# fishaudio/Bert-VITS2

Hardware: AMD Instinct MI355X
Metric: audio-seconds/sec (44.1 kHz), SynthesizerTrn.infer(), 128-phoneme utterance (higher is better)
Workload: dtype f32; 1 GPU; BASELINE config 2: B=1 x T=128 symbols per GPU, fp32 Generator (split-bf16 MFMA), fp32 flow, fp32 text encoder / durations / spline; utterances_per_gpu=1, symbols=128, frames=384, parallelism=utterance-sharded x1, hipgraph=False, hip_force_dev_kernarg=1

## Files before the change

### bert-vits2_amd/csrc/bv2_kernels.h

```cpp
#pragma once
#include <hip/hip_runtime_api.h>
#include <stdint.h>
#include <map>
#include <mutex>
#include <utility>

namespace bv2 {

#if defined(__HIPCC__)
__device__ __forceinline__ bool xcd_decode(unsigned id, int per, int B, int& b, int& r) {
  const unsigned slot = id >> 3;
  b = (int)(slot / (unsigned)per) * 8 + (int)(id & 7u);
  r = (int)(slot % (unsigned)per);
  return b < B;
}
#endif
inline int xcd_grid(int B, int per) { return 8 * ((B + 7) / 8) * per; }

struct Prefetch { const void* ptr; unsigned bytes; };
constexpr int PF_BLOCKS = 128;
#if defined(__HIPCC__)
__device__ __forceinline__ void prefetch_tail(const Prefetch pf, unsigned l, unsigned j, unsigned tid, unsigned nthreads) {
  const unsigned lines = (pf.bytes + 127u) >> 7;
  const unsigned lx = (lines + 7u) >> 3;
// ... 53 lines not shown
  int act;
  int mask_pre;
  int res_mode;
  int mask_post;
  const uint16_t* w3;
  const float* w3inv;
  const unsigned* xmax;
  unsigned* omax;
};

#define BV2_MAX_PROBS 8
#define BV2_MAX_KSPLIT 8
struct ConvLaunch {
  ConvProb p[BV2_MAX_PROBS];
  int nprob;
  int B;
  int L;
  const int64_t* lens = nullptr; int len_mul = 1;
  int ksplit;
  int64_t slab_stride;
  unsigned long long* dbg = nullptr;
  Prefetch pf = {nullptr, 0};
  int no_head = 0;
};

struct ConvLaunch1 {
  ConvProb p;
  int L; int64_t slab_stride; unsigned long long* dbg;
};
struct SkHead {
  const float* x; const float* w; const float* in_mask;
  int x_rstride, Lin, ntiles, per_xcd, total;
  unsigned pk0, pk1;
};
struct SkSmall { int k, dil, pad_left, ksplit, cin, cin_pad; };
#if defined(__HIPCC__)
#define BV2_HD __host__ __device__
#else
#define BV2_HD
#endif
BV2_HD inline SkSmall sk_head_unpack(unsigned pk0, unsigned pk1) {
  return SkSmall{(int)(pk0 & 255u), (int)((pk0 >> 8) & 255u), (int)((pk0 >> 16) & 255u), (int)(pk0 >> 24), (int)(pk1 & 65535u), (int)(pk1 >> 16)};
}
inline bool sk_head_pack(const ConvLaunch& L, int ntiles, int per_xcd, int total, SkHead* h) {
  const ConvProb& p = L.p[0];
  if (L.no_head || L.nprob != 1 || L.B != 1 || L.lens || p.nsrc != 1 || (L.pf.ptr && L.pf.bytes)) return false;
  if (p.k < 1 || p.k > 255 || p.dil < 1 || p.dil > 255 || p.pad_left < 0 || p.pad_left > 255 || L.ksplit < 1 || L.ksplit > 255) return false;
  if (p.cin < 1 || p.cin > 65535 || p.cin_pad < 1 || p.cin_pad > 65535) return false;
  h->x = p.x[0]; h->w = p.w; h->in_mask = p.in_mask;
  h->x_rstride = p.x_rstride; h->Lin = p.Lin; h->ntiles = ntiles; h->per_xcd = per_xcd; h->total = total;
  h->pk0 = (unsigned)p.k | (unsigned)p.dil << 8 | (unsigned)p.pad_left << 16 | (unsigned)L.ksplit << 24;
  h->pk1 = (unsigned)p.cin | (unsigned)p.cin_pad << 16;
  return true;
}
void conv_set_timeline(unsigned long long* dev_buf, long long capacity_u64);
int conv_timeline_report(long long* meta, int max_launches);
unsigned long long* timeline_slice(unsigned gx, unsigned gy, unsigned gz, int tile, int ks, int cin, int L);

enum { TILE_AUTO = 0, TILE_128x128 = 1, TILE_64x128 = 2, TILE_64x64 = 3, TILE_32x128 = 4, TILE_32x256 = 5, TILE_SPLITK = 6, TILE_128x64 = 7,
       TILE_X6 = 8,
       TILE_X6_128x64 = 9, TILE_X6_128x64_LD = 10, TILE_X6_64x128 = 11, TILE_X6_32x256 = 12,
       TILE_X3 = 14 };
int launch_conv1d(hipStream_t stream, const ConvLaunch& L, int tile, const char** variant_name);
enum { PLACE_PLAIN = 0, PLACE_PER_XCD = 1, PLACE_SNAKE = 2 };
void conv_note_placement(int place);
int conv_last_placement();
inline int64_t x6_w_index(int j, int ci, int co, int cin, int k, int plane) {
  const int64_t U = (int64_t)(cin / 16) * k, u = (int64_t)(ci / 16) * k + j;
  const int lane = (co & 31) + 32 * ((ci % 16) / 8);
  return ((((int64_t)(co >> 5) * U + u) * 3 + plane) * 64 + lane) * 8 + (ci % 8);
}
inline int64_t x6_w_elems(int cin, int cout_pad, int k) { return (int64_t)(cout_pad / 32) * (cin / 16) * k * 3 * 512; }
inline uint16_t f2bf(float f) {
  uint32_t u;
  __builtin_memcpy(&u, &f, 4);
  if ((u & 0x7fffffffu) > 0x7f800000u) return (uint16_t)((u >> 16) | 0x40u);
  u += 0x7fffu + ((u >> 16) & 1u);
  return (uint16_t)(u >> 16);
}
inline uint16_t f2h(float f) {
  const _Float16 h = (_Float16)f;
  uint16_t u;
  __builtin_memcpy(&u, &h, 2);
  return u;
}
inline float h2f(uint16_t u) {
  _Float16 h;
  __builtin_memcpy(&h, &u, 2);
  return (float)h;
}
inline void x6_split(float v, uint16_t h[3]) {
  for (int p = 0; p < 3; ++p) {
    uint32_t u;
    __builtin_memcpy(&u, &v, 4);
    uint16_t b;
    if ((u & 0x7fffffffu) > 0x7f800000u) b = (uint16_t)((u >> 16) | 0x40u);
    else if (p == 0 && (u & 0x7fffffffu) > 0x7f7f0000u) b = (uint16_t)((u >> 16) & 0x8000u) | 0x7f7fu;
    else { u += 0x7fffu + ((u >> 16) & 1u); b = (uint16_t)(u >> 16); }
    h[p] = b;
// ... 512 lines not shown
```

### bert-vits2_amd/csrc/bv2_testing.cpp

```cpp
#include <cmath>
#include <cstddef>
#include <cstring>
#include <vector>

#include "bv2_internal.h"
#include "bv2_pack.h"
#include "../../include/bv2_testing.h"
#include "kernels/rng.h"

using namespace bv2;

static auto t_dense(const float* w, int cin, int k) {
  return [=](int co, int ci, int j) { return w[((size_t)co * cin + ci) * k + j]; };
}
static auto t_bias(const float* b) { return [=](int co) { return b ? b[co] : 0.f; }; }

extern "C" {

int64_t bv2_test_conv_pack_floats(int cin, int cout, int k) {
  const ConvW c = conv_desc(cin, cout, k);
  const int64_t base = conv_w_floats(c) + c.cout_pad + 2048;
  return base + (cin % 32 == 0 ? x6_w_floats(c) + 64 + 2 * X3_SLOT_WORDS + x3_region_floats(c) + 64 : 0);
}
void bv2_test_x6_split(float v, uint16_t* h3) { x6_split(v, h3); }
// ... 507 lines not shown
                          float* out, int B, int H, int D, int T, int P, int span) {
  DebertaAttnArgs a;
  a.qkv = qkv; a.ld = ld; a.mask = mask; a.pk = pk; a.pq = pq; a.tab = tab; a.out = out;
  a.B = B; a.H = H; a.D = D; a.T = T; a.P = P; a.span = span;
  return launch_deberta_attn(static_cast<hipStream_t>(stream), a);
}

int bv2_test_bert_ln(void* stream, const float* a, int nslab, int64_t slab_stride, const float* gamma, const float* beta, float eps,
                     const float* mask, float* out, int B, int C, int T, const void* pf_ptr, unsigned pf_bytes) {
  BertLnArgs l;
  l.a = a; l.nslab = nslab; l.slab_stride = slab_stride; l.gamma = gamma; l.beta = beta; l.eps = eps; l.mask = mask; l.out = out;
  l.B = B; l.C = C; l.T = T;
  l.pf = Prefetch{pf_ptr, pf_bytes};
  return launch_bert_ln(static_cast<hipStream_t>(stream), l);
}

int bv2_test_bert_embed_ln(void* stream, const int64_t* input_ids, const int64_t* token_type_ids, const float* word, const float* pos,
                           const float* type, const int64_t* lengths, const float* gamma, const float* beta, float eps, float* out,
                           int B, int S, int C, int vocab, int max_pos, int type_vocab, const void* pf_ptr, unsigned pf_bytes) {
  BertEmbedArgs e;
  e.input_ids = input_ids; e.token_type_ids = token_type_ids; e.word = word; e.pos = pos; e.type = type; e.lengths = lengths;
  e.gamma = gamma; e.beta = beta; e.eps = eps; e.out = out;
  e.B = B; e.S = S; e.C = C; e.vocab = vocab; e.max_pos = max_pos; e.type_vocab = type_vocab;
  e.pf = Prefetch{pf_ptr, pf_bytes};
  return launch_bert_embed_ln(static_cast<hipStream_t>(stream), e);
}

void bv2_test_conv_timeline(void* dev_buf, long long capacity_u64) {
  conv_set_timeline(static_cast<unsigned long long*>(dev_buf), capacity_u64);
}
int bv2_test_conv_timeline_report(long long* meta, int max_launches) { return conv_timeline_report(meta, max_launches); }

void bv2_test_set_tuning(int splitk_waves, int force_ck, long tile_target) { conv_set_tuning(splitk_waves, force_ck, tile_target); }
void bv2_test_set_x6_tuning(int t256, int t128, int t64, int ck) { conv_x6_set_tuning(t256, t128, t64, ck); }
void bv2_test_x6_occupancy(int* out4) { conv_x6_occupancy(out4); }
void bv2_test_set_variants(const char* cl_spec, int cl_generic, int hc_generic) {
  conv_cl_set_tuning(cl_spec, cl_generic);
  conv_f16_set_tuning(hc_generic);
}

int64_t bv2_test_dds_pack_floats(int C) {
  return 10 * (int64_t)C + 2 * bv2_test_conv_pack_floats(C, C, 1);
}

int bv2_test_dds_layer(void* stream, const float* x, const float* pre_w_host, const float* pre_b_host, const float* z, int z_src,
                       const float* g, const float* mask, const float* dww_host, const float* dwb_host, const float* g1_host,
                       const float* b1_host, const float* g2_host, const float* b2_host, const float* w_host,
                       const float* bias_host, float* out, int dil, int last_mask, const float* post_w_host,
                       const float* post_b_host, int post_cout, float* post_out, float* zio, int z_dst, float* wpack_dev,
                       int B, int C, int T) {
  try {
    const int64_t one = bv2_test_conv_pack_floats(C, C, 1);
    std::vector<float> pk((size_t)bv2_test_dds_pack_floats(C), 0.f);
    size_t o = 0;
    auto put = [&](const float* src, size_t n) { size_t at = o; if (src) std::memcpy(&pk[o], src, n * sizeof(float)); o += n; return at; };
    const size_t o_dww = put(dww_host, 3 * (size_t)C), o_dwb = put(dwb_host, C), o_g1 = put(g1_host, C), o_b1 = put(b1_host, C),
                 o_g2 = put(g2_host, C), o_b2 = put(b2_host, C), o_pw = put(pre_w_host, C), o_pb = put(pre_b_host, C);
    const size_t o_w = o, boff = (size_t)conv_w_floats(conv_desc(C, C, 1));
    t_pack_conv(&pk[o_w], w_host, bias_host, C, C, 1, false);
    const size_t o_p = o_w + (size_t)one;
    if (post_w_host) {
      pack_f32(&pk[o_p], C, post_cout, 1, t_dense(post_w_host, C, 1));
      if (post_b_host) pack_bias(&pk[o_p + boff], post_cout, t_bias(post_b_host));
    }
    if (hipMemcpy(wpack_dev, pk.data(), sizeof(float) * pk.size(), hipMemcpyHostToDevice) != hipSuccess) return -6;
    DdsArgs a;
// ... 193 lines not shown
```

### bert-vits2_amd/csrc/kernels/attention.hip

```cpp
#include <hip/hip_runtime.h>
#include <type_traits>
#include <math.h>
#include "device_helpers.h"

namespace bv2 {

constexpr int AQ_WIDE = 32;
constexpr int AQ_NARROW = 16;
constexpr int AK = 32;
constexpr int ATTN_CUS = 256;
constexpr int AMAXW = 8;
constexpr int ANS = 4;


struct AttnHead { const float* qkv; const float* mask; const float* erv; int ld, T, H, W, ksplit; };

template <int DT, int NW, bool F16, bool ONE, bool KV16, int QT>
__device__ __forceinline__ void attention_tile(const AttnHead Hd, const AttnArgs& A, const int b, const int h, const int bx,
                                               const unsigned long long ts0) {
  static_assert(!KV16 || F16, "fp16 K / V only feed the fp16 matrix products");
  static_assert(QT == AQ_WIDE || (QT == AQ_NARROW && !F16), "the fp16 forms stay on 32 queries");
  constexpr int D = 32 * DT;
  constexpr int NT = 64 * NW;
  constexpr int AQ = QT, QSH = QT == 32 ? 5 : 4;
// ... 602 lines not shown
  if (ntiles <= 8 && !(DT == 4 && qt == AQ_NARROW)) return launch_attn_variant<DT, 8, true>(stream, a, grid, qt);
  if constexpr (DT == 4) return launch_attn_variant<DT, 4, false>(stream, a, grid, qt);
  else return launch_attn_variant<DT, 8, false>(stream, a, grid, qt);
}

int attention_pick_qtile(int B, int H, int T, int D, int ksplit, bool f16) {
  if (f16 || D < 32 || D > 128 || D % 32) return AQ_WIDE;
  const int ks = ksplit > 1 ? ksplit : 1, qtiles = (T + AQ_WIDE - 1) / AQ_WIDE;
  return (long)B * H * qtiles * ks * 2 <= ATTN_CUS ? AQ_NARROW : AQ_WIDE;
}

int launch_attention(hipStream_t stream, const AttnArgs& a) {
  if (a.W > AMAXW || a.W < 0 || a.T < 1 || a.B < 1 || a.H < 1 || a.ld % 32 || a.ld < a.T) return -1;
  if ((a.kh != nullptr) != (a.vh != nullptr) || (a.kh && !a.f16)) return -1;
  if (a.wo && (a.f16 || !a.o_out || a.Co < 1 || a.wo_groups * 8 < a.H * a.D)) return -1;
  if ((a.qtile != 0 && a.qtile != AQ_NARROW && a.qtile != AQ_WIDE) || (a.qtile == AQ_NARROW && a.f16)) return -1;
  const int ks = a.ksplit > 1 ? a.ksplit : 1;
  const int ntiles_all = (a.T + AK - 1) / AK;
  if (ks > 1 && (!a.wo || !a.ml_out || a.bo || a.res || ks > ntiles_all)) return -1;
  const int qt = a.qtile ? a.qtile : attention_pick_qtile(a.B, a.H, a.T, a.D, ks, a.f16 != 0);
  dim3 grid(((a.T + qt - 1) / qt) * ks, a.H, a.B);
  const int ntiles = (ntiles_all + ks - 1) / ks;
  switch (a.D) {
    case 32: return launch_attn_d<1>(stream, a, grid, ntiles, qt);
    case 64: return launch_attn_d<2>(stream, a, grid, ntiles, qt);
    case 96: return launch_attn_d<3>(stream, a, grid, ntiles, qt);
    case 128: return launch_attn_d<4>(stream, a, grid, ntiles, qt);
    default: return -2;
  }
}

int attention_pick_ksplit(int B, int H, int T, int max_slabs) {
  const int ntiles = (T + AK - 1) / AK;
  if (ntiles <= 8 || H < 1 || (H & (H - 1))) return 1;
  int ks = 1;
  auto wgs = [&](int k) {
    const int qt = attention_pick_qtile(B, H, T, 32, k, false);
    return (long)B * H * ((T + qt - 1) / qt) * k;
  };
  while (ks * 4 < ntiles && H * ks * 2 <= max_slabs && H * ks * 2 <= 8 && wgs(ks * 2) <= 512) ks *= 2;
  return ks;
}

double attention_flops(const AttnArgs& a) {
  return (double)a.B * a.H * (4.0 * a.T * (double)a.T * a.D);
}

}
```

### bert-vits2_amd/csrc/kernels/conv_mfma.hip

```cpp
#include <hip/hip_runtime.h>
#include "device_helpers.h"

namespace bv2 {

template <int WM, int WN, int MI, int NI, int CK, int XS>
__global__ void __launch_bounds__(256) conv1d_mfma_kernel(const ConvLaunch L, const int mtiles, const int per_xcd, const int snake_n) {
  constexpr int BM = WM * MI * 32;
  constexpr int BN = WN * NI * 32;
  constexpr int XP = XS * 64;
  constexpr int RPW = CK / 4;
  constexpr int GR = CK / 8;
  static_assert(WM * WN == 4, "4 waves per workgroup");
  extern __shared__ __attribute__((aligned(16))) float smem[];

  int pz = blockIdx.z, by = blockIdx.y, bx = blockIdx.x;
  if (snake_n > 0) {
    const int xcd = blockIdx.x & 7, pp = blockIdx.x >> 3;
    if (pp >= snake_n) return;
    const int r = pp >> 5, cc = pp & 31;
    const int rem = snake_n - (r << 5) < 32 ? snake_n - (r << 5) : 32;
    const int sidx = (r << 5) + ((r & 1) ? rem - 1 - cc : cc);
    const int per_prob = per_xcd * mtiles * L.B;
    pz = sidx / per_prob;
    const int rest = sidx - pz * per_prob;
// ... 245 lines not shown
        }
#pragma unroll
        for (int r = 0; r < 16; ++r) {
          const int dr = (r & 3) + 8 * (r >> 2);
          float v = acc[mi][ni][r] + bsum(r);
          if (act == ACT_RELU) v = v < 0.f ? 0.f : v;
          else if (act == ACT_GELU) v = 0.5f * v * (1.0f + erff(v * 0.70710678118654752440f));
          if (mask_pre) v *= om;
          if (res_mode == RES_ADD) v += rv[r];
          else if (res_mode == RES_RSUB) v = rv[r] - v;
          if (mask_post) v *= om;
          if (colok && row0 + dr < cout) {
            outb[off0 + (unsigned)dr * o_rs] = v;
            vmx = fmaxf(vmx, fabsf(v));
          }
        }
      }
    }
    if (omax_w) x3_publish(omax_w, omax_seen, vmx, lane);
  }
  if (L.dbg && tid == 0) {
    __builtin_amdgcn_s_waitcnt(0);
    unsigned long long* d = L.dbg + 8ull * (snake_n > 0 ? (unsigned long long)blockIdx.x
                                                        : ((unsigned long long)blockIdx.z * gridDim.y + blockIdx.y) * gridDim.x + blockIdx.x);
    timeline_record(d, ts0, ts1, ts2, k);
  }
}

constexpr int SK_PD = 8;


constexpr int SK_XP = 64;
constexpr int SK_RPW = 32;
struct SkTile {
  int nt, z, mt, b, ksplit;
  const float* xp; const float* mp; const float* wp;
  int x_rstride, Lin, k, dil, pad_left, cin, cin_pad;
};

template <bool MASK, int NWV, bool LDSX>
__device__ __forceinline__ void splitk_tile(float* const red_raw, const SkTile S, const ConvProb& P, const int L_L, const int64_t slab_stride,
                                            unsigned long long* const dbg, const unsigned long long ts0) {
  float (*red)[32][33] = reinterpret_cast<float (*)[32][33]>(red_raw);
  unsigned long long ts1 = 0, ts2 = 0;
  const int nt = S.nt, z = S.z, mt = S.mt, b = S.b;
  const int m0 = mt * 32, t0 = nt * 32;

  const int tid = threadIdx.x;
  const int lane = tid & 63;
  const int wid = __builtin_amdgcn_readfirstlane(tid >> 6);
  const int l31 = lane & 31, lh = lane >> 5;
  const int k = S.k, dil = S.dil, cin = S.cin, Lin = S.Lin;
  const int groups = S.cin_pad / 8;
  const float* const xp = S.xp;
  const float* const mp = MASK ? S.mp : nullptr;
  const float* const wp = S.wp;
  const unsigned x_rs4 = 4u * (unsigned)S.x_rstride;
  const unsigned w_tap = 1024u;
  const unsigned w_unit = w_tap * (unsigned)k;
  const unsigned w_lane = 16u * (unsigned)(lh * 32 + l31) + (unsigned)mt * (unsigned)groups * w_unit;
  const unsigned nsl = (unsigned)(S.ksplit * NWV), sl = (unsigned)(z * NWV + wid);
  const int g0 = (int)(((unsigned)groups * sl) / nsl), g1 = (int)(((unsigned)groups * (sl + 1u)) / nsl);
  const int U = (g1 - g0) * k;

  f32x16 acc, acc2;
#pragma unroll
  for (int r = 0; r < 16; ++r) { acc[r] = 0.f; acc2[r] = 0.f; }

  const int tcol = t0 + l31 - S.pad_left;
  f32x4 ar[SK_PD];
  float br[SK_PD][4];
  float mr[SK_PD];
  bool vmr[SK_PD];
// ... 5 lines not shown
    const int gc = g < groups ? g : groups - 1;
    return (unsigned)(8 * gc + lh) * x_rs4;
  };
  auto weight_off = [&](int g) __attribute__((always_inline)) {
    const int gc = g < groups ? g : groups - 1;
    return w_lane + (unsigned)gc * w_unit;
  };
  unsigned goff = group_off(lg), woff = weight_off(lg), joff = 0;
  auto load_unit = [&](int slot) __attribute__((always_inline)) {
    ar[slot] = ld_off4(wp, woff + joff);
    if (LDSX) {
      joff += w_tap;
      if (++lj == k) { lj = 0; joff = 0; ++lg; woff = weight_off(lg); }
      return;
    }
    const int t = tcol + lj * dil;
    const bool tok = t >= 0 && t < Lin;
    const unsigned tcl = 4u * (unsigned)(t < 0 ? 0 : (t >= Lin ? Lin - 1 : t));
    vmr[slot] = tok;
    mr[slot] = MASK ? ld_off(mp, tcl) : 1.f;
    unsigned ro = goff;
#pragma unroll
    for (int q = 0; q < 4; ++q) {
      const unsigned rc = ro < row_max ? ro : row_max;
      br[slot][q] = ld_off(xp, rc + tcl);
      ro += x_rs8;
    }
    joff += w_tap;
    if (++lj == k) { lj = 0; joff = 0; ++lg; goff = group_off(lg); woff = weight_off(lg); }
  };

  const int G0 = (int)(((unsigned)groups * (unsigned)(z * NWV)) / nsl);
  float* const Xs = red_raw;
  float xv[LDSX ? SK_RPW : 1];
  float mval = 1.f;
  bool xtok = false;
  if (LDSX) {
    const int XW = 32 + (k - 1) * dil;
    const int t = t0 - S.pad_left + lane;
    xtok = lane < XW && t >= 0 && t < Lin;
    const unsigned tcl = 4u * (unsigned)(t < 0 ? 0 : (t >= Lin ? Lin - 1 : t));
    if (MASK) mval = ld_off(mp, tcl);
#pragma unroll
    for (int i = 0; i < SK_RPW; ++i) {
      int row = 8 * G0 + wid + NWV * i;
      row = row < cin ? row : cin - 1;
      xv[i] = ld_off(xp, (unsigned)row * x_rs4 + tcl);
    }
  }
#pragma unroll
  for (int i = 0; i < SK_PD; ++i) { load_unit(i); __builtin_amdgcn_sched_barrier(0); }

  asm volatile("" ::"s"(P.in_scale), "s"(P.slope), "s"(P.pre_act), "s"(P.cout), "s"(P.act), "s"(P.mask_pre), "s"(P.mask_post), "s"(P.res_mode),
               "s"(P.out_rstride), "s"(P.out_tstride), "s"(P.out_toff), "s"(P.out), "s"(P.out_bstride), "s"(P.res), "s"(P.res_bstride),
               "s"(P.bias), "s"(P.bias2), "s"(P.bias2_bstride), "s"(P.out_mask), "s"(P.out_mask_bstride), "s"(P.omax), "s"(L_L),
               "s"(slab_stride), "s"(dbg));
  const float in_scale = P.in_scale, slope = P.slope;
  const bool pre_lrelu = P.pre_act == PRE_LRELU;
  const int col = t0 + (tid & 31);
  const bool colok = col < L_L;
  const int cout = P.cout, act = P.act, mask_pre = P.mask_pre, mask_post = P.mask_post, res_mode = P.res_mode;
  const unsigned o_rs = (unsigned)P.out_rstride, o_ts = (unsigned)P.out_tstride, o_to = (unsigned)P.out_toff;
  float* const outb = P.out + (int64_t)z * slab_stride + (int64_t)b * P.out_bstride;
  const float* const resb = (res_mode != RES_NONE && z == 0) ? P.res + (int64_t)b * P.res_bstride : nullptr;
  const float* const biasp = z == 0 ? P.bias : nullptr;
  const float* const bias2p = (z == 0 && P.bias2) ? P.bias2 + (int64_t)b * P.bias2_bstride : nullptr;
  const float om = (P.out_mask && colok) ? P.out_mask[(int64_t)b * P.out_mask_bstride + col] : 1.f;
  unsigned* const omaxp = P.omax ? x3_slot_word(P.omax) : nullptr;
  const unsigned coff = (unsigned)(colok ? col : 0) * o_ts + o_to;
  constexpr int RPP = 2 * NWV;
  float rvv[32 / RPP], bsv[32 / RPP], b2v[32 / RPP];
#pragma unroll
  for (int i = 0; i < 32 / RPP; ++i) {
    const int rl = (tid >> 5) + RPP * i;
    int row = m0 + rl;
    row = row < cout ? row : cout - 1;
    bsv[i] = biasp ? biasp[row] : 0.f;
    b2v[i] = bias2p ? bias2p[row] : 0.f;
    rvv[i] = resb ? ld_off(resb, 4u * ((unsigned)row * o_rs + coff)) : 0.f;
  }
  if (LDSX) {
    const int G1 = (int)(((unsigned)groups * (unsigned)((z + 1) * NWV)) / nsl);
    const int nrows = 8 * (G1 - G0);
    const float cs = xtok ? in_scale * mval : 0.f;
#pragma unroll
    for (int i = 0; i < SK_RPW; ++i) {
      const int rr = wid + NWV * i;
      float x = xv[i];
      const float xn = x * slope;
      x = (pre_lrelu && x < 0.f) ? xn : x;
      Xs[rr * SK_XP + lane] = (rr < nrows && 8 * G0 + rr < cin) ? x * cs : 0.f;
    }
  }
  if (LDSX) __syncthreads();
  if (dbg) ts1 = __builtin_amdgcn_s_memtime();
  if (LDSX) {
    int ug = g0, uj = 0;
    float bq[2][4];
    {
      const float* xb = Xs + (8 * (ug - G0) + lh) * SK_XP + l31;
#pragma unroll
      for (int q = 0; q < 4; ++q) bq[0][q] = xb[q * 2 * SK_XP];
    }
    for (int u0 = 0; u0 < U; u0 += SK_PD) {
#pragma unroll
      for (int i = 0; i < SK_PD; ++i) {
        if (u0 + i < U) {
          int jn = uj + 1, gn = ug;
          if (jn == k) { jn = 0; ++gn; }
          const bool more = u0 + i + 1 < U;
          const float* xb = Xs + (8 * ((more ? gn : ug) - G0) + lh) * SK_XP + l31 + (more ? jn : uj) * dil;
#pragma unroll
          for (int q = 0; q < 4; ++q) bq[(i & 1) ^ 1][q] = xb[q * 2 * SK_XP];
          acc = __builtin_amdgcn_mfma_f32_32x32x2f32(ar[i].x, bq[i & 1][0], acc, 0, 0, 0);
          acc2 = __builtin_amdgcn_mfma_f32_32x32x2f32(ar[i].y, bq[i & 1][1], acc2, 0, 0, 0);
          acc = __builtin_amdgcn_mfma_f32_32x32x2f32(ar[i].z, bq[i & 1][2], acc, 0, 0, 0);
          acc2 = __builtin_amdgcn_mfma_f32_32x32x2f32(ar[i].w, bq[i & 1][3], acc2, 0, 0, 0);
// ... 89 lines not shown
}

template <bool MASK, int NWV, bool LDSX>
__global__ void __launch_bounds__(64 * NWV) conv1d_splitk_kernel(const ConvLaunch L, const int mtiles, const int ntiles,
                                                                 const int per_xcd, const int total) {
  extern __shared__ __attribute__((aligned(16))) float red_raw[];
  const int bid = blockIdx.x;
  if (bid >= per_xcd * 8) {
    prefetch_tail(L.pf, (unsigned)bid, (unsigned)(bid - per_xcd * 8), threadIdx.x, 64 * NWV);
    return;
  }
  unsigned long long ts0 = 0;
  if (L.dbg) ts0 = __builtin_amdgcn_s_memtime();
  const int v = (bid & 7) * per_xcd + (bid >> 3);
  if (v >= total) return;
  int rem = v;
  SkTile S;
  S.nt = rem % ntiles; rem /= ntiles;
  S.z = rem % L.ksplit; rem /= L.ksplit;
  S.mt = rem % mtiles; rem /= mtiles;
  S.b = rem % L.B; rem /= L.B;
  S.ksplit = L.ksplit;
  const ConvProb P = L.p[rem];
  if (S.mt * 32 >= P.cout_pad) return;
  S.Lin = P.Lin;
  if (L.lens) {
    const int64_t lv = L.lens[S.b] * L.len_mul;
    S.Lin = lv < S.Lin ? (int)lv : S.Lin;
  }
  S.xp = P.x[0] + (int64_t)S.b * P.x_bstride;
  S.mp = MASK ? P.in_mask + (int64_t)S.b * P.in_mask_bstride : nullptr;
  S.wp = P.w;
  S.x_rstride = P.x_rstride; S.k = P.k; S.dil = P.dil; S.pad_left = P.pad_left; S.cin = P.cin; S.cin_pad = P.cin_pad;
  splitk_tile<MASK, NWV, LDSX>(red_raw, S, P, L.L, L.slab_stride, L.dbg, ts0);
}

template <bool MASK, int NWV, bool LDSX>
__global__ void __launch_bounds__(64 * NWV) conv1d_splitk1_kernel(const float* const x, const float* const w, const float* const in_mask,
                                                                  const int x_rstride, const int Lin, const int ntiles, const int per_xcd,
                                                                  const int total, const unsigned pk0, const unsigned pk1,
                                                                  const ConvLaunch1 L) {
  extern __shared__ __attribute__((aligned(16))) float red_raw[];
  const int bid = blockIdx.x;
  const unsigned long long ts0 = __builtin_amdgcn_s_memtime();
  const int v = (bid & 7) * per_xcd + (bid >> 3);
  if (v >= total) return;
  const SkSmall q = sk_head_unpack(pk0, pk1);
  int rem = v;
  SkTile S;
  S.nt = rem % ntiles; rem /= ntiles;
  S.z = rem % q.ksplit; rem /= q.ksplit;
  S.mt = rem;
  S.b = 0; S.ksplit = q.ksplit;
  S.xp = x; S.mp = in_mask; S.wp = w;
  S.x_rstride = x_rstride; S.Lin = Lin; S.k = q.k; S.dil = q.dil; S.pad_left = q.pad_left; S.cin = q.cin; S.cin_pad = q.cin_pad;
  splitk_tile<MASK, NWV, LDSX>(red_raw, S, L.p, L.L, L.slab_stride, L.dbg, ts0);
}

struct TileCfg { int id, bm, bn, xs; const char* name; };
static const TileCfg kTiles[] = {
    {TILE_128x128, 128, 128, 3, "conv1d_mfma<128x128>"}, {TILE_64x128, 64, 128, 3, "conv1d_mfma<64x128>"},
    {TILE_32x256, 32, 256, 5, "conv1d_mfma<32x256>"},    {TILE_64x64, 64, 64, 2, "conv1d_mfma<64x64>"},
    {TILE_32x128, 32, 128, 3, "conv1d_mfma<32x128>"},
};
static const TileCfg kTile128x64 = {TILE_128x64, 128, 64, 2, "conv1d_mfma<128x64>"};

static int g_tune_splitk_waves = 0, g_tune_force_ck = 0, g_tune_no_ldsx = 0, g_tune_no_snake = 0;
static long g_tune_tile_target = 0;
void conv_set_tuning(int splitk_waves, int force_ck, long tile_target) {
  g_tune_no_ldsx = splitk_waves >= 100 ? 1 : 0;
  g_tune_splitk_waves = splitk_waves % 100; g_tune_force_ck = force_ck % 100; g_tune_tile_target = tile_target;
  g_tune_no_snake = force_ck >= 100 ? 1 : 0;
}

static int g_last_placement = PLACE_PLAIN;
void conv_note_placement(int place) { g_last_placement = place; }
int conv_last_placement() { return g_last_placement; }

static unsigned long long* g_tl_buf = nullptr;
static long long g_tl_cap = 0, g_tl_off = 0;
struct TlMeta { long long off; int gx, gy, gz, tile, ks, cin, L; };
static TlMeta g_tl_meta[512];
static int g_tl_n = 0;
void conv_set_timeline(unsigned long long* dev_buf, long long capacity_u64) { g_tl_buf = dev_buf; g_tl_cap = capacity_u64; g_tl_off = 0; g_tl_n = 0; }
int conv_timeline_report(long long* meta, int max_launches) {
  int n = g_tl_n < max_launches ? g_tl_n : max_launches;
  for (int i = 0; i < n; ++i) {
    const TlMeta& m = g_tl_meta[i];
    long long* o = meta + 8 * i;
    o[0] = m.off; o[1] = m.gx; o[2] = m.gy; o[3] = m.gz; o[4] = m.tile; o[5] = m.ks; o[6] = m.cin; o[7] = m.L;
  }
  return n;
}
unsigned long long* timeline_slice(unsigned gx, unsigned gy, unsigned gz, int tile, int ks, int cin, int L) {
  if (!g_tl_buf) return nullptr;
  const long long need = 8ll * gx * gy * gz;
  if (g_tl_off + need > g_tl_cap || g_tl_n >= 512) return nullptr;
  unsigned long long* r = g_tl_buf + g_tl_off;
  g_tl_meta[g_tl_n++] = TlMeta{g_tl_off, (int)gx, (int)gy, (int)gz, tile, ks, cin, L};
  g_tl_off += need;
  return r;
}
static ConvLaunch with_timeline(const ConvLaunch& L, dim3 grid, int tile) {
  ConvLaunch r = L;
  if (!g_tl_buf) return r;
  int ks = 0;
  for (int i = 0; i < L.nprob && i < 3; ++i) ks |= (L.p[i].k & 255) << (8 * i);
  r.dbg = timeline_slice(grid.x, grid.y, grid.z, tile, ks, L.p[0].cin, L.L);
  return r;
}
// ... 38 lines not shown
  return hipGetLastError() == hipSuccess ? 0 : -1;
}

constexpr int SK_UNITS_PER_WAVE = 16;

static int splitk_units(const ConvLaunch& L) {
  int units = 0;
  for (int i = 0; i < L.nprob; ++i) {
    const int u = (L.p[i].cin_pad / 8) * L.p[i].k;
    if (u > units) units = u;
  }
  return units;
}

static int splitk_waves(const ConvLaunch& L) {
  if (g_tune_splitk_waves == 4 || g_tune_splitk_waves == 8 || g_tune_splitk_waves == 16) return g_tune_splitk_waves;
  const int slices = (splitk_units(L) + SK_UNITS_PER_WAVE - 1) / SK_UNITS_PER_WAVE;
  const int per_wg = (slices + L.ksplit - 1) / L.ksplit;
  return per_wg > 4 ? 8 : 4;
}

static int splitk_stage_rows(const ConvLaunch& L, int nw) {
  int rows = 0;
  for (int i = 0; i < L.nprob; ++i) {
    const int groups = L.p[i].cin_pad / 8, nsl = L.ksplit * nw;
    for (int z = 0; z < L.ksplit; ++z) {
      const int a = (int)(((int64_t)groups * (z * nw)) / nsl), b = (int)(((int64_t)groups * ((z + 1) * nw)) / nsl);
      rows = 8 * (b - a) > rows ? 8 * (b - a) : rows;
    }
  }
  return rows;
}

template <bool MASK, bool LDSX>
static void launch_splitk_nw(hipStream_t stream, const ConvLaunch& L, int nw, dim3 grid, int mtiles, int ntiles, int per_xcd,
                             int total, int stage_rows) {
  size_t lds = sizeof(float) * (size_t)nw * 32 * 33;
  if (LDSX) lds = sizeof(float) * (size_t)nw * SK_RPW * SK_XP;
  (void)stage_rows;
  SkHead h;
  if (nw <= 8 && sk_head_pack(L, ntiles, per_xcd, total, &h)) {
    const ConvLaunch1 L1{L.p[0], L.L, L.slab_stride, L.dbg};
    if (nw == 8) {
      auto kern = conv1d_splitk1_kernel<MASK, 8, LDSX>;
      ensure_dyn_lds((const void*)kern, lds);
      hipLaunchKernelGGL(kern, grid, dim3(512), lds, stream, h.x, h.w, h.in_mask, h.x_rstride, h.Lin, h.ntiles, h.per_xcd, h.total,
                         h.pk0, h.pk1, L1);
    } else {
      auto kern = conv1d_splitk1_kernel<MASK, 4, LDSX>;
      ensure_dyn_lds((const void*)kern, lds);
      hipLaunchKernelGGL(kern, grid, dim3(256), lds, stream, h.x, h.w, h.in_mask, h.x_rstride, h.Lin, h.ntiles, h.per_xcd, h.total,
                         h.pk0, h.pk1, L1);
    }
    return;
  }
  if (nw == 16) {
    auto kern = conv1d_splitk_kernel<MASK, 16, LDSX>;
    ensure_dyn_lds((const void*)kern, lds);
    hipLaunchKernelGGL(kern, grid, dim3(1024), lds, stream, L, mtiles, ntiles, per_xcd, total);
  } else if (nw == 8) {
    auto kern = conv1d_splitk_kernel<MASK, 8, LDSX>;
    ensure_dyn_lds((const void*)kern, lds);
    hipLaunchKernelGGL(kern, grid, dim3(512), lds, stream, L, mtiles, ntiles, per_xcd, total);
  } else {
    auto kern = conv1d_splitk_kernel<MASK, 4, LDSX>;
    ensure_dyn_lds((const void*)kern, lds);
    hipLaunchKernelGGL(kern, grid, dim3(256), lds, stream, L, mtiles, ntiles, per_xcd, total);
  }
}

static int launch_splitk(hipStream_t stream, const ConvLaunch& L0, int max_cout_pad, const char** variant_name) {
  const int mtiles = max_cout_pad / 32, ntiles = (L0.L + 31) / 32;
  const ConvLaunch L = with_timeline(L0, dim3(((L0.nprob * L0.B * mtiles * L0.ksplit * ntiles + 7) / 8) * 8), 32032);
  const int total = L.nprob * L.B * mtiles * L.ksplit * ntiles;
  const int per_xcd = (total + 7) / 8;
  bool any_mask = false, all_mask = true;
  for (int i = 0; i < L.nprob; ++i) {
    if (L.p[i].nsrc != 1) return -2;
    if (L.p[i].in_mask) any_mask = true; else all_mask = false;
  }
  if (any_mask != all_mask) return -2;
  int nw = splitk_waves(L);
  for (int i = 0; i < L.nprob; ++i)
    if (L.p[i].act == ACT_GATE && nw == 16) nw = 8;
  if (variant_name) *variant_name = nw == 16 ? "conv1d_splitk<32x32,16w>" : (nw == 8 ? "conv1d_splitk<32x32,8w>" : "conv1d_splitk<32x32,4w>");
  const dim3 grid(per_xcd * 8 + (L.pf.ptr && L.pf.bytes ? PF_BLOCKS : 0));
  conv_note_placement(PLACE_PER_XCD);
  bool ldsx = !g_tune_no_ldsx;
// ... 128 lines not shown
```

### include/bv2_testing.h

```cpp
#ifndef BV2_TESTING_H
#define BV2_TESTING_H
#include <stdint.h>
#include "bv2.h"
#ifdef __cplusplus
extern "C" {
#endif

int64_t bv2_test_conv_pack_floats(int cin, int cout, int k);

int bv2_test_conv1d(void* stream, const float* x, const float* w_host, const float* bias_host, float* out, float* wpack_dev,
                    int B, int cin, int cout, int k, int dil, int pad_left, int L, int tile, float lrelu_slope, int relu,
                    const float* res, int res_mode, const float* in_mask, const float* out_mask, int mask_pre,
                    int mask_post, const float* bias2, int nsrc, const float* x1, const float* x2, float in_scale, int ksplit,
                    int64_t slab_stride);


int64_t bv2_test_x3_omax_off(int cin, int cout, int k);

void bv2_test_x6_split(float v, uint16_t* h3);
int bv2_test_convert(int kind, const void* in, void* out, int64_t n);
int bv2_test_x6_regions(const bv2_handle* h, int64_t* off_floats, int64_t* n_floats, int max_regions);
int bv2_test_x3_regions(const bv2_handle* h, int64_t* off_floats, int64_t* n_floats, int max_regions);

int bv2_test_resblock_fused(void* stream, const float* x, float* out, const float* w1_host, const float* b1_host,
// ... 73 lines not shown
                       const float* post_b_host, int post_cout, float* post_out, float* zio, int z_dst, float* wpack_dev,
                       int B, int C, int T);


int bv2_test_ups_split(int u, int k, int cin, int cout, const float* w, float* phase_w, int32_t* pad_left, float* cl_w, int32_t* cl_dims,
                       int32_t* cl_offs);

typedef struct bv2_test_conv_prob {
  const float* w_host; const float* bias_host;
  int32_t k, dil, pad_left;
  float* out; int32_t out_rstride, out_tstride, out_toff;
  const float* res; int32_t res_mode;
} bv2_test_conv_prob;
int64_t bv2_test_conv_multi_pack_floats(int cin, int cout, const int32_t* k, int nprob);
int bv2_test_conv_multi(void* stream, const bv2_test_conv_prob* probs, int nprob, int cin, int cout, const float* x0, const float* x1,
                        const float* x2, int nsrc, float in_scale, float lrelu_slope, const int64_t* lens, int len_mul, int B, int L,
                        int tile, int ksplit, int64_t slab_stride, const float* out_mask, unsigned* omax, float* wpack_dev, int32_t* info);

int64_t bv2_test_conv_transpose_pack_floats(int u, int k, int cin, int cout);
int bv2_test_conv_transpose(void* stream, const float* w_host, const float* bias_host, int u, int k, int cin, int cout, const float* x0,
                            const float* x1, const float* x2, int nsrc, float* out, const int64_t* lens, int len_mul, int B, int L,
                            int tile, int only_phase, unsigned* omax, float* wpack_dev, int32_t* info);
int64_t bv2_test_conv_transpose_cl_pack_bytes(int u, int k, int cin, int cout);
int bv2_test_conv_transpose_cl(void* stream, const float* w_host, const float* bias_host, int u, int k, int cin, int cout, const void* x0,
                               const void* x1, const void* x2, int nsrc, void* out, const int64_t* lens, int len_mul, int B, int L,
                               int phase_taps, void* wpack_dev);

int bv2_test_conv_post(void* stream, const float* x0, const float* x1, const float* x2, int nsrc, const float* w_host, float* w_dev,
                       float* out, const int64_t* lens, int len_mul, int B, int C, int k, int L);
int bv2_test_conv_post_cl(void* stream, const void* x0, const void* x1, const void* x2, int nsrc, const float* w_host, float* w_dev,
                          float* out, const int64_t* lens, int len_mul, int B, int C, int k, int L, int generic);

void bv2_test_set_tuning(int splitk_waves, int force_ck, long tile_target);
void bv2_test_set_kernarg_head(int on);
int bv2_test_splitk_head(int k, int dil, int pad_left, int ksplit, int cin, int cin_pad, int B, int has_lens, int nprob, int32_t* out6);
void bv2_test_set_x6_tuning(int t256, int t128, int t64, int ck);
void bv2_test_x6_occupancy(int* out4);
void bv2_test_set_variants(const char* cl_spec, int cl_generic, int hc_generic);

void bv2_test_conv_timeline(void* dev_buf, long long capacity_u64);
int bv2_test_conv_timeline_report(long long* meta, int max_launches);

int bv2_test_spline(void* stream, float* z, int src, int dst, const float* params, int prow, const float* mask,
                    float sqrt_fc, float tail, int B, int T);

int bv2_test_spline_forward(void* stream, const float* x, const float* uw, const float* uh, const float* ud, float tail, long long N,
                            float* y, float* logabsdet);

void bv2_test_philox4x32_10(const uint32_t ctr[4], const uint32_t key[2], uint32_t out[4]);
float bv2_test_seeded_normal(int64_t seed, int which, int row, int t);

#ifdef __cplusplus
}
#endif
#endif
```

Before: 1679 audio-seconds/sec.

## Stage split-K conv input rows across all threads and split attention keys for short sequences

The split-K conv head kernel gains an EPT template path. It maps threads over a (row, column) grid of the input window, so each thread loads 16 or 24 rows instead of 32 lanes-per-wave loads that leave lanes idle when the window is narrow. Rows that fall outside the window go to an extra dump row in LDS. Separately, attention picks a key split of 2 for the B=1, 4-tile case to get more workgroups on short sequences. The changes add template instances and reciprocal-multiply row indexing, which could be wrong for edge widths, plus an extra reduction for the attention split.

```diff
diff --git a/bert-vits2_amd/csrc/bv2_kernels.h b/bert-vits2_amd/csrc/bv2_kernels.h
--- a/bert-vits2_amd/csrc/bv2_kernels.h
+++ b/bert-vits2_amd/csrc/bv2_kernels.h
@@ -109,6 +109,7 @@
   const float* x; const float* w; const float* in_mask;
   int x_rstride, Lin, ntiles, per_xcd, total;
   unsigned pk0, pk1;
+  unsigned pk2 = 0;
 };
 struct SkSmall { int k, dil, pad_left, ksplit, cin, cin_pad; };
 #if defined(__HIPCC__)
@@ -142,6 +143,7 @@
 enum { PLACE_PLAIN = 0, PLACE_PER_XCD = 1, PLACE_SNAKE = 2 };
 void conv_note_placement(int place);
 int conv_last_placement();
+int conv_last_splitk_stage();
 inline int64_t x6_w_index(int j, int ci, int co, int cin, int k, int plane) {
   const int64_t U = (int64_t)(cin / 16) * k, u = (int64_t)(ci / 16) * k + j;
   const int lane = (co & 31) + 32 * ((ci % 16) / 8);
diff --git a/bert-vits2_amd/csrc/bv2_testing.cpp b/bert-vits2_amd/csrc/bv2_testing.cpp
--- a/bert-vits2_amd/csrc/bv2_testing.cpp
+++ b/bert-vits2_amd/csrc/bv2_testing.cpp
@@ -563,6 +563,7 @@
 int bv2_test_conv_timeline_report(long long* meta, int max_launches) { return conv_timeline_report(meta, max_launches); }
 
 void bv2_test_set_tuning(int splitk_waves, int force_ck, long tile_target) { conv_set_tuning(splitk_waves, force_ck, tile_target); }
+int bv2_test_splitk_stage(void) { return conv_last_splitk_stage(); }
 void bv2_test_set_x6_tuning(int t256, int t128, int t64, int ck) { conv_x6_set_tuning(t256, t128, t64, ck); }
 void bv2_test_x6_occupancy(int* out4) { conv_x6_occupancy(out4); }
 void bv2_test_set_variants(const char* cl_spec, int cl_generic, int hc_generic) {
diff --git a/bert-vits2_amd/csrc/kernels/attention.hip b/bert-vits2_amd/csrc/kernels/attention.hip
--- a/bert-vits2_amd/csrc/kernels/attention.hip
+++ b/bert-vits2_amd/csrc/kernels/attention.hip
@@ -658,7 +658,9 @@
 
 int attention_pick_ksplit(int B, int H, int T, int max_slabs) {
   const int ntiles = (T + AK - 1) / AK;
-  if (ntiles <= 8 || H < 1 || (H & (H - 1))) return 1;
+  if (H < 1 || (H & (H - 1))) return 1;
+  if (ntiles == 4 && B == 1 && H * 2 <= max_slabs && H * 2 <= 8) return 2;
+  if (ntiles <= 8) return 1;
   int ks = 1;
   auto wgs = [&](int k) {
     const int qt = attention_pick_qtile(B, H, T, 32, k, false);
diff --git a/bert-vits2_amd/csrc/kernels/conv_mfma.hip b/bert-vits2_amd/csrc/kernels/conv_mfma.hip
--- a/bert-vits2_amd/csrc/kernels/conv_mfma.hip
+++ b/bert-vits2_amd/csrc/kernels/conv_mfma.hip
@@ -301,13 +301,15 @@
 
 constexpr int SK_XP = 64;
 constexpr int SK_RPW = 32;
+constexpr int SK_DUMP = 1;
 struct SkTile {
   int nt, z, mt, b, ksplit;
   const float* xp; const float* mp; const float* wp;
   int x_rstride, Lin, k, dil, pad_left, cin, cin_pad;
+  unsigned st_mul; int st_rpp;
 };
 
-template <bool MASK, int NWV, bool LDSX>
+template <bool MASK, int NWV, bool LDSX, int EPT = 0>
 __device__ __forceinline__ void splitk_tile(float* const red_raw, const SkTile S, const ConvProb& P, const int L_L, const int64_t slab_stride,
                                             unsigned long long* const dbg, const unsigned long long ts0) {
   float (*red)[32][33] = reinterpret_cast<float (*)[32][33]>(red_raw);
@@ -379,20 +381,33 @@
 
   const int G0 = (int)(((unsigned)groups * (unsigned)(z * NWV)) / nsl);
   float* const Xs = red_raw;
-  float xv[LDSX ? SK_RPW : 1];
+  constexpr int XN = LDSX ? (EPT ? EPT : SK_RPW) : 1;
+  float xv[XN];
   float mval = 1.f;
   bool xtok = false;
+  const int sr0 = EPT ? (int)(((unsigned)tid * S.st_mul) >> 16) : 0;
+  const int sc = EPT ? tid - sr0 * (32 + (k - 1) * dil) : lane;
   if (LDSX) {
     const int XW = 32 + (k - 1) * dil;
-    const int t = t0 - S.pad_left + lane;
-    xtok = lane < XW && t >= 0 && t < Lin;
+    const int t = t0 - S.pad_left + sc;
+    xtok = sc < XW && t >= 0 && t < Lin;
     const unsigned tcl = 4u * (unsigned)(t < 0 ? 0 : (t >= Lin ? Lin - 1 : t));
     if (MASK) mval = ld_off(mp, tcl);
-#pragma unroll
-    for (int i = 0; i < SK_RPW; ++i) {
-      int row = 8 * G0 + wid + NWV * i;
-      row = row < cin ? row : cin - 1;
-      xv[i] = ld_off(xp, (unsigned)row * x_rs4 + tcl);
+    if constexpr (EPT > 0) {
+      int row = 8 * G0 + sr0;
+#pragma unroll
+      for (int i = 0; i < EPT; ++i) {
+        const int rc = row < cin ? row : cin - 1;
+        xv[i] = ld_off(xp, (unsigned)rc * x_rs4 + tcl);
+        row += S.st_rpp;
+      }
+    } else {
+#pragma unroll
+      for (int i = 0; i < SK_RPW; ++i) {
+        int row = 8 * G0 + wid + NWV * i;
+        row = row < cin ? row : cin - 1;
+        xv[i] = ld_off(xp, (unsigned)row * x_rs4 + tcl);
+      }
     }
   }
 #pragma unroll
@@ -430,6 +445,19 @@
     const int G1 = (int)(((unsigned)groups * (unsigned)((z + 1) * NWV)) / nsl);
     const int nrows = 8 * (G1 - G0);
     const float cs = xtok ? in_scale * mval : 0.f;
+    if constexpr (EPT > 0) {
+      const bool mine = sr0 < S.st_rpp;
+      int rr = sr0;
+#pragma unroll
+      for (int i = 0; i < EPT; ++i) {
+        float x = xv[i];
+        const float xn = x * slope;
+        x = (pre_lrelu && x < 0.f) ? xn : x;
+        const bool ok = mine && rr < nrows;
+        Xs[(ok ? rr : 32 * NWV) * SK_XP + sc] = (ok && 8 * G0 + rr < cin) ? x * cs : 0.f;
+        rr += S.st_rpp;
+      }
+    } else
 #pragma unroll
     for (int i = 0; i < SK_RPW; ++i) {
       const int rr = wid + NWV * i;
@@ -585,13 +613,14 @@
   S.mp = MASK ? P.in_mask + (int64_t)S.b * P.in_mask_bstride : nullptr;
   S.wp = P.w;
   S.x_rstride = P.x_rstride; S.k = P.k; S.dil = P.dil; S.pad_left = P.pad_left; S.cin = P.cin; S.cin_pad = P.cin_pad;
+  S.st_mul = 0; S.st_rpp = 0;
   splitk_tile<MASK, NWV, LDSX>(red_raw, S, P, L.L, L.slab_stride, L.dbg, ts0);
 }
 
-template <bool MASK, int NWV, bool LDSX>
+template <bool MASK, int NWV, bool LDSX, int EPT>
 __global__ void __launch_bounds__(64 * NWV) conv1d_splitk1_kernel(const float* const x, const float* const w, const float* const in_mask,
                                                                   const int x_rstride, const int Lin, const int ntiles, const int per_xcd,
-                                                                  const int total, const unsigned pk0, const unsigned pk1,
+                                                                  const int total, const unsigned pk0, const unsigned pk1, const unsigned pk2,
                                                                   const ConvLaunch1 L) {
   extern __shared__ __attribute__((aligned(16))) float red_raw[];
   const int bid = blockIdx.x;
@@ -607,7 +636,8 @@
   S.b = 0; S.ksplit = q.ksplit;
   S.xp = x; S.mp = in_mask; S.wp = w;
   S.x_rstride = x_rstride; S.Lin = Lin; S.k = q.k; S.dil = q.dil; S.pad_left = q.pad_left; S.cin = q.cin; S.cin_pad = q.cin_pad;
-  splitk_tile<MASK, NWV, LDSX>(red_raw, S, L.p, L.L, L.slab_stride, L.dbg, ts0);
+  S.st_mul = pk2 & 65535u; S.st_rpp = (int)(pk2 >> 16);
+  splitk_tile<MASK, NWV, LDSX, EPT>(red_raw, S, L.p, L.L, L.slab_stride, L.dbg, ts0);
 }
 
 struct TileCfg { int id, bm, bn, xs; const char* name; };
@@ -618,10 +648,11 @@
 };
 static const TileCfg kTile128x64 = {TILE_128x64, 128, 64, 2, "conv1d_mfma<128x64>"};
 
-static int g_tune_splitk_waves = 0, g_tune_force_ck = 0, g_tune_no_ldsx = 0, g_tune_no_snake = 0;
+static int g_tune_splitk_waves = 0, g_tune_force_ck = 0, g_tune_no_ldsx = 0, g_tune_no_snake = 0, g_tune_row_stage = 0;
 static long g_tune_tile_target = 0;
 void conv_set_tuning(int splitk_waves, int force_ck, long tile_target) {
-  g_tune_no_ldsx = splitk_waves >= 100 ? 1 : 0;
+  g_tune_no_ldsx = splitk_waves >= 100 && splitk_waves < 200 ? 1 : 0;
+  g_tune_row_stage = splitk_waves >= 200 ? 1 : 0;
   g_tune_splitk_waves = splitk_waves % 100; g_tune_force_ck = force_ck % 100; g_tune_tile_target = tile_target;
   g_tune_no_snake = force_ck >= 100 ? 1 : 0;
 }
@@ -629,6 +660,8 @@
 static int g_last_placement = PLACE_PLAIN;
 void conv_note_placement(int place) { g_last_placement = place; }
 int conv_last_placement() { return g_last_placement; }
+static int g_last_splitk_stage = -1;
+int conv_last_splitk_stage() { return g_last_splitk_stage; }
 
 static unsigned long long* g_tl_buf = nullptr;
 static long long g_tl_cap = 0, g_tl_off = 0;
@@ -733,28 +766,43 @@
   return rows;
 }
 
+template <bool MASK, int NWV, bool LDSX, int EPT>
+static void launch_splitk_head(hipStream_t stream, dim3 grid, size_t lds, const SkHead& h, const ConvLaunch1& L1) {
+  auto kern = conv1d_splitk1_kernel<MASK, NWV, LDSX, EPT>;
+  ensure_dyn_lds((const void*)kern, lds);
+  hipLaunchKernelGGL(kern, grid, dim3(64 * NWV), lds, stream, h.x, h.w, h.in_mask, h.x_rstride, h.Lin, h.ntiles, h.per_xcd, h.total,
+                     h.pk0, h.pk1, h.pk2, L1);
+}
+template <bool MASK, int NWV, bool LDSX>
+static void launch_splitk_head_ept(hipStream_t stream, dim3 grid, size_t lds, const SkHead& h, const ConvLaunch1& L1, int ept) {
+  if constexpr (LDSX) {
+    if (ept == 16) return launch_splitk_head<MASK, NWV, true, 16>(stream, grid, lds, h, L1);
+    if (ept == 24) return launch_splitk_head<MASK, NWV, true, 24>(stream, grid, lds, h, L1);
+  }
+  launch_splitk_head<MASK, NWV, LDSX, 0>(stream, grid, lds, h, L1);
+}
+
 template <bool MASK, bool LDSX>
 static void launch_splitk_nw(hipStream_t stream, const ConvLaunch& L, int nw, dim3 grid, int mtiles, int ntiles, int per_xcd,
                              int total, int stage_rows) {
   size_t lds = sizeof(float) * (size_t)nw * 32 * 33;
-  if (LDSX) lds = sizeof(float) * (size_t)nw * SK_RPW * SK_XP;
-  (void)stage_rows;
+  if (LDSX) lds = sizeof(float) * (size_t)(nw * SK_RPW + SK_DUMP) * SK_XP;
   SkHead h;
   if (nw <= 8 && sk_head_pack(L, ntiles, per_xcd, total, &h)) {
     const ConvLaunch1 L1{L.p[0], L.L, L.slab_stride, L.dbg};
-    if (nw == 8) {
-      auto kern = conv1d_splitk1_kernel<MASK, 8, LDSX>;
-      ensure_dyn_lds((const void*)kern, lds);
-      hipLaunchKernelGGL(kern, grid, dim3(512), lds, stream, h.x, h.w, h.in_mask, h.x_rstride, h.Lin, h.ntiles, h.per_xcd, h.total,
-                         h.pk0, h.pk1, L1);
-    } else {
-      auto kern = conv1d_splitk1_kernel<MASK, 4, LDSX>;
-      ensure_dyn_lds((const void*)kern, lds);
-      hipLaunchKernelGGL(kern, grid, dim3(256), lds, stream, h.x, h.w, h.in_mask, h.x_rstride, h.Lin, h.ntiles, h.per_xcd, h.total,
-                         h.pk0, h.pk1, L1);
-    }
+    int ept = 0;
+    if (LDSX && !g_tune_row_stage) {
+      const int xw = 32 + (L.p[0].k - 1) * L.p[0].dil, rpp = 64 * nw / xw;
+      const int need = (stage_rows + rpp - 1) / rpp;
+      ept = need <= 16 ? 16 : (need <= 24 ? 24 : 0);
+      h.pk2 = (unsigned)(65536 / xw + 1) | (unsigned)rpp << 16;
+    }
+    g_last_splitk_stage = LDSX ? ept : -1;
+    if (nw == 8) launch_splitk_head_ept<MASK, 8, LDSX>(stream, grid, lds, h, L1, ept);
+    else launch_splitk_head_ept<MASK, 4, LDSX>(stream, grid, lds, h, L1, ept);
     return;
   }
+  g_last_splitk_stage = LDSX ? 0 : -1;
   if (nw == 16) {
     auto kern = conv1d_splitk_kernel<MASK, 16, LDSX>;
     ensure_dyn_lds((const void*)kern, lds);
diff --git a/include/bv2_testing.h b/include/bv2_testing.h
--- a/include/bv2_testing.h
+++ b/include/bv2_testing.h
@@ -129,6 +129,7 @@
                           float* out, const int64_t* lens, int len_mul, int B, int C, int k, int L, int generic);
 
 void bv2_test_set_tuning(int splitk_waves, int force_ck, long tile_target);
+int bv2_test_splitk_stage(void);
 void bv2_test_set_kernarg_head(int on);
 int bv2_test_splitk_head(int k, int dil, int pad_left, int ksplit, int cin, int cin_pad, int B, int has_lens, int nprob, int32_t* out6);
 void bv2_test_set_x6_tuning(int t256, int t128, int t64, int ck);
```

Measured after the change: 1711 audio-seconds/sec, median of 6. 1.02x the previous value.
